# thu-ml/stochastic_gcn

Measured on AMD Instinct MI355X. Metric: training edges/s (SpMM), higher is better.
Workload: dtype f32

## Files before the change

### stochastic_gcn_amd/csrc/sgcn_gemm.hip

```cpp
#include "sgcn_dev.h"
#include "sgcn_bwd.h"

namespace sgcn {

typedef float f16acc __attribute__((ext_vector_type(16)));

constexpr int kTM = 32, kTN = 128, kTK = 32;

struct GemmArgs {
    const float* A; int64_t lda;
    const float* B; int64_t ldb;
    float* C; int64_t ldc;
    int32_t M, N, K;
    int32_t accumulate;
    int32_t kchunk;
    float* ws;
    const float* offset; const float* scale; float eps; int32_t relu;
    float* xhat; float* rstd;
    int32_t epi;
    const float* A2; int64_t lda2; int32_t a_split;
    DropArgs drop_a;
    DropArgs drop_c;
    int32_t vec_a, vec_b;
    const int32_t* a_gidx;
    const int32_t* a_gidx2;
};

__device__ __forceinline__ float wsum(float v) {
#pragma unroll
    for (int o = 32; o > 0; o >>= 1) v += __shfl_xor(v, o, 64);
    return v;
}

constexpr int kAsFloats = kTM * (kTK + 1), kBsFloats = kTK * (kTN + 4);
constexpr int kGroupFloats = kAsFloats + kBsFloats;

template <bool TA, bool TB, int KG>
__device__ __forceinline__ void gemm_body(const GemmArgs& g, const int bx, const int by, const int bz) {
    extern __shared__ float smem[];
    const int kg = threadIdx.x / kBlock;
    const int tid = threadIdx.x % kBlock, lane = tid & 63, wave = tid >> 6;
    float (*As)[kTK + 1] = reinterpret_cast<float (*)[kTK + 1]>(smem + kg * kGroupFloats);
    float (*Bs)[kTN + 4] = reinterpret_cast<float (*)[kTN + 4]>(smem + kg * kGroupFloats + kAsFloats);
    const int m0 = bx * kTM, n0 = by * kTN;
    const int kbeg = bz * g.kchunk;
    const int kend = min(g.K, kbeg + g.kchunk);
    f16acc acc = {};
    float ra[4], rb[16];
    float ep_scale[2] = {1.f, 1.f}, ep_offset[2] = {0.f, 0.f};
    if (g.epi == 2) {
#pragma unroll
        for (int e = 0; e < 2; e++) {
            const int c = (threadIdx.x & 63) + e * kWave;
            if (c < g.N) { ep_scale[e] = g.scale[c]; ep_offset[e] = g.offset[c]; }
        }
    }

    auto ld4 = [&](const float* rowp, bool vec, bool rowok, int first, int limit, float* out) {
        if (vec) {
            const bool ok = rowok && first + 3 < limit;
            const float4 v = *reinterpret_cast<const float4*>(rowp + (ok ? first : 0));
            out[0] = ok ? v.x : 0.f; out[1] = ok ? v.y : 0.f; out[2] = ok ? v.z : 0.f; out[3] = ok ? v.w : 0.f;
        } else {
#pragma unroll
            for (int e = 0; e < 4; e++) {
                const bool ok = rowok && first + e < limit;
                const float v = rowp[ok ? first + e : 0];
                out[e] = ok ? v : 0.f;
            }
        }
    };
    const float* arow = nullptr;
    if (!TA) {
        const int row = min(m0 + (tid >> 3), g.M - 1);
        if (g.A2 && row >= g.a_split) {
            const int r2 = row - g.a_split;
            arow = g.A2 + (int64_t)(g.a_gidx2 ? g.a_gidx2[r2] : r2) * g.lda2;
        } else {
            arow = g.A + (int64_t)(g.a_gidx ? g.a_gidx[row] : row) * g.lda;
        }
    }
    auto fetch = [&](int k0) {
        if (!TA) {
            const int i = tid >> 3, kq = (tid & 7) * 4, row = m0 + i;
            ld4(arow, g.vec_a, row < g.M, k0 + kq, kend, ra);
            if (g.drop_a.on) {
#pragma unroll
                for (int e = 0; e < 4; e++) ra[e] *= drop_factor(g.drop_a, row, k0 + kq + e);
            }
        } else {
            const int kk = tid >> 3, iq = (tid & 7) * 4, k = k0 + kk, kc = min(k, kend - 1);
            const int64_t ak = g.a_gidx ? g.a_gidx[kc] : kc;
            ld4(g.A + ak * g.lda, g.vec_a, k < kend, m0 + iq, g.M, ra);
            if (g.drop_a.on) {
#pragma unroll
                for (int e = 0; e < 4; e++) ra[e] *= drop_factor(g.drop_a, k, m0 + iq + e);
            }
        }
        if (!TB) {
#pragma unroll
            for (int r = 0; r < 4; r++) {
                const int kk = (tid >> 5) + 8 * r, jq = (tid & 31) * 4, k = k0 + kk;
                ld4(g.B + (int64_t)min(k, kend - 1) * g.ldb, g.vec_b, k < kend, n0 + jq, g.N, rb + r * 4);
            }
        } else {
#pragma unroll
            for (int r = 0; r < 4; r++) {
                const int j = (tid >> 3) + 32 * r, kq = (tid & 7) * 4, col = n0 + j;
                ld4(g.B + (int64_t)min(col, g.N - 1) * g.ldb, g.vec_b, col < g.N, k0 + kq, kend, rb + r * 4);
            }
        }
    };
    auto stage = [&]() {
        if (!TA) {
            const int i = tid >> 3, kq = (tid & 7) * 4;
#pragma unroll
            for (int e = 0; e < 4; e++) As[i][kq + e] = ra[e];
        } else {
            const int kk = tid >> 3, iq = (tid & 7) * 4;
#pragma unroll
            for (int e = 0; e < 4; e++) As[iq + e][kk] = ra[e];
        }
        if (!TB) {
#pragma unroll
            for (int r = 0; r < 4; r++) {
                const int kk = (tid >> 5) + 8 * r, jq = (tid & 31) * 4;
                *reinterpret_cast<float4*>(&Bs[kk][jq]) = make_float4(rb[r * 4], rb[r * 4 + 1], rb[r * 4 + 2], rb[r * 4 + 3]);
            }
        } else {
#pragma unroll
            for (int r = 0; r < 4; r++) {
                const int j = (tid >> 3) + 32 * r, kq = (tid & 7) * 4;
#pragma unroll
                for (int e = 0; e < 4; e++) Bs[kq + e][j] = rb[r * 4 + e];
            }
        }
    };

    const int iters = ((kend - kbeg + kTK - 1) / kTK + KG - 1) / KG;
    if (iters > 0) fetch(kbeg + kg * kTK);
    for (int it = 0; it < iters; it++) {
        const int k0 = kbeg + (it * KG + kg) * kTK;
        stage();
        __syncthreads();
        if (it + 1 < iters) fetch(k0 + KG * kTK);
        const int fi = lane & 31, fk = lane >> 5;
#pragma unroll
        for (int kk2 = 0; kk2 < kTK / 2; kk2++) {
            const float a = As[fi][kk2 * 2 + fk];
            const float b = Bs[kk2 * 2 + fk][wave * 32 + fi];
            acc = __builtin_amdgcn_mfma_f32_32x32x2f32(a, b, acc, 0, 0, 0);
        }
        __syncthreads();
    }

    const int cj = wave * 32 + (lane & 31);
    if (KG > 1) {
        if (kg > 0) {
#pragma unroll
            for (int r = 0; r < 16; r++) Bs[(r & 3) + 8 * (r >> 2) + 4 * (lane >> 5)][cj] = acc[r];
        }
        __syncthreads();
        if (kg == 0) {
            for (int o = 1; o < KG; o++) {
                float (*P)[kTN + 4] = reinterpret_cast<float (*)[kTN + 4]>(smem + o * kGroupFloats + kAsFloats);
#pragma unroll
                for (int r = 0; r < 16; r++) acc[r] += P[(r & 3) + 8 * (r >> 2) + 4 * (lane >> 5)][cj];
            }
        }
    }
    if (g.epi == 0) {
        if (kg != 0) return;
        float* base = g.ws ? g.ws + (int64_t)bz * g.M * g.N : g.C;
        const int64_t ld = g.ws ? g.N : g.ldc;
        const bool add = !g.ws && g.accumulate;
#pragma unroll
        for (int r = 0; r < 16; r++) {
            const int row = m0 + (r & 3) + 8 * (r >> 2) + 4 * (lane >> 5), col = n0 + cj;
            if (row < g.M && col < g.N) {
                float* p = base + (int64_t)row * ld + col;
                float v = acc[r];
                if (g.drop_c.on) v *= drop_factor(g.drop_c, row, col);
                *p = add ? *p + v : v;
            }
        }
        return;
    }
    float (*Cs)[kTN + 4] = reinterpret_cast<float (*)[kTN + 4]>(smem + kAsFloats);
    if (KG > 1) __syncthreads();
    if (kg == 0) {
#pragma unroll
        for (int r = 0; r < 16; r++) Cs[(r & 3) + 8 * (r >> 2) + 4 * (lane >> 5)][cj] = acc[r];
    }
    __syncthreads();
    for (int rr = kg * (kBlock / kWave) + wave; rr < kTM; rr += KG * (kBlock / kWave)) {
        const int row = m0 + rr;
        if (row >= g.M) break;
        float* yr = g.C + (int64_t)row * g.ldc;
        if (g.epi == 1) {
            for (int c = lane; c < g.N; c += kWave) { const float v = Cs[rr][c]; yr[c] = g.relu ? fmaxf(v, 0.f) : v; }
            continue;
        }
        float s = 0.f;
        for (int c = lane; c < g.N; c += kWave) s += Cs[rr][c];
        const float mean = wsum(s) / (float)g.N;
        float q = 0.f;
        for (int c = lane; c < g.N; c += kWave) { const float t = Cs[rr][c] - mean; q += t * t; }
        const float rs = rsqrtf(wsum(q) / (float)g.N + g.eps);
        if (lane == 0) g.rstd[row] = rs;
        float* hr = g.xhat + (int64_t)row * g.N;
#pragma unroll
        for (int e = 0; e < 2; e++) {
            const int c = lane + e * kWave;
            if (c < g.N) {
                const float h = (Cs[rr][c] - mean) * rs;
                hr[c] = h;
                const float v = h * ep_scale[e] + ep_offset[e];
                yr[c] = g.relu ? fmaxf(v, 0.f) : v;
            }
        }
    }
}

template <bool TA, bool TB, int KG>
__global__ __launch_bounds__(kBlock * KG) void gemm_kernel(GemmArgs g) {
    gemm_body<TA, TB, KG>(g, (int)blockIdx.x, (int)blockIdx.y, (int)blockIdx.z);
}

struct GemmGroup {
    GemmArgs g[kMaxGroup];
    int32_t first[kMaxGroup + 1];
    int32_t gx[kMaxGroup], gy[kMaxGroup];
    int32_t n;
};

template <bool TA, bool TB, int KG>
__global__ __launch_bounds__(kBlock * KG) void gemm_group_kernel(GemmGroup G) {
    const int b = (int)blockIdx.x;
    int j = 0;
#pragma unroll
    for (int q = 1; q < kMaxGroup; q++) j += (q < G.n && b >= G.first[q]) ? 1 : 0;
    const int l = b - G.first[j];
    const int gx = G.gx[j], gy = G.gy[j];
    gemm_body<TA, TB, KG>(G.g[j], l % gx, (l / gx) % gy, l / (gx * gy));
}

__global__ void splitk_reduce_kernel(const float* __restrict__ ws, int32_t S, int32_t M, int32_t N,
                                     float* __restrict__ C, int64_t ldc, int32_t accumulate) {
    const int64_t i = (int64_t)blockIdx.x * blockDim.x + threadIdx.x;
    const int64_t mn = (int64_t)M * N;
    if (i >= mn) return;
    float s = 0.f;
    for (int z = 0; z < S; z++) s += ws[(int64_t)z * mn + i];
    float* p = C + (i / N) * ldc + (i % N);
    *p = accumulate ? *p + s : s;
}

__global__ void dense_bwd_reduce_kernel(ReduceJob j, int32_t gemm_blocks, const float* __restrict__ ln_partial,
                                        int32_t nblk, int32_t d, float* __restrict__ doffset,
                                        float* __restrict__ dscale, int32_t ln_accumulate) {
    if ((int)blockIdx.x < gemm_blocks) {
        const int64_t i = (int64_t)blockIdx.x * blockDim.x + threadIdx.x;
        const int64_t mn = (int64_t)j.M * j.N;
        if (i >= mn) return;
        float s = 0.f;
        for (int z = 0; z < j.S; z++) s += j.ws[(int64_t)z * mn + i];
        float* p = j.C + (i / j.N) * j.ldc + (i % j.N);
        *p = j.accumulate ? *p + s : s;
    } else {
        ln_param_reduce_cols32(ln_partial, nblk, d, doffset, dscale, (int)blockIdx.x - gemm_blocks, ln_accumulate != 0);
    }
}

__global__ void dense_bwd_reduce_multi_kernel(ReduceMulti R) { reduce_multi_body(R, (int)blockIdx.x, nullptr); }

__global__ __launch_bounds__(kBlock) void splitk_ln_act_kernel(const float* __restrict__ ws, int32_t S,
                                                               GemmArgs g) {
    const int lane = threadIdx.x & 63;
    const int64_t row = (int64_t)blockIdx.x * (kBlock / kWave) + threadIdx.x / kWave;
    if (row >= g.M) return;
    const int64_t mn = (int64_t)g.M * g.N;
    float v[2];
    float sc[2] = {1.f, 1.f}, of[2] = {0.f, 0.f};
    if (g.epi == 2) {
#pragma unroll
        for (int e = 0; e < 2; e++) {
            const int c = lane + e * kWave;
            if (c < g.N) { sc[e] = g.scale[c]; of[e] = g.offset[c]; }
        }
    }
#pragma unroll
    for (int e = 0; e < 2; e++) {
        const int c = lane + e * kWave;
        float s = 0.f;
        if (c < g.N)
            for (int z = 0; z < S; z++) s += ws[(int64_t)z * mn + row * g.N + c];
        v[e] = s;
    }
    float* yr = g.C + row * g.ldc;
    if (g.epi == 2) {
        const float mean = wsum(v[0] + v[1]) / (float)g.N;
        float q = 0.f;
#pragma unroll
        for (int e = 0; e < 2; e++) if (lane + e * kWave < g.N) { const float t = v[e] - mean; q += t * t; }
// ... 93 lines not shown
    }
    if (d.drop.on) { x[0] *= drop_factor(d.drop, (int)row, lane); x[1] *= drop_factor(d.drop, (int)row, lane + kWave); }
    const int c0 = lane < d.N ? lane : 0, c1 = lane + kWave < d.N ? lane + kWave : 0;
    float a0[2] = {0.f, 0.f}, a1[2] = {0.f, 0.f};
    for (int s0 = 0; s0 * 32 < K2; s0++) {
        const int gi = d.kg > 1 ? (s0 & 1) : 0;
        const float xs = s0 < 2 ? x[0] : x[1];
        const int kb = s0 * 32, lb = kb & (kWave - 1);
        const float* wk = wl + kb * d.N;
        float p0 = a0[gi], p1 = a1[gi];
        if (kb + 32 <= K2) {
#pragma unroll
            for (int q = 0; q < 4; q++) {
                float w0[8], w1[8];
#pragma unroll
                for (int u = 0; u < 8; u++) { w0[u] = wk[(q * 8 + u) * d.N + c0]; w1[u] = wk[(q * 8 + u) * d.N + c1]; }
#pragma unroll
                for (int u = 0; u < 8; u++) {
                    const float xv = __int_as_float(__builtin_amdgcn_readlane(__float_as_int(xs), lb + q * 8 + u));
                    p0 = fmaf(xv, w0[u], p0); p1 = fmaf(xv, w1[u], p1);
                }
            }
        } else {
            for (int kk = 0; kb + kk < K2; kk++) {
                const float xv = __int_as_float(__builtin_amdgcn_readlane(__float_as_int(xs), lb + kk));
                p0 = fmaf(xv, wk[kk * d.N + c0], p0); p1 = fmaf(xv, wk[kk * d.N + c1], p1);
            }
        }
        a0[gi] = p0; a1[gi] = p1;
    }
    const float z[2] = {d.kg > 1 ? a0[0] + a0[1] : a0[0], d.kg > 1 ? a1[0] + a1[1] : a1[0]};
    float* y2 = d.Y + row * d.ldy;
    if (d.epi != 2) {
#pragma unroll
        for (int e = 0; e < 2; e++) {
            const int c = lane + e * kWave;
            if (c < d.N) y2[c] = (d.epi == 1 && d.relu) ? fmaxf(z[e], 0.f) : z[e];
        }
        return;
    }
    float s = 0.f;
#pragma unroll
    for (int e = 0; e < 2; e++) if (lane + e * kWave < d.N) s += z[e];
    const float mean = wsum(s) / (float)d.N;
    float q = 0.f;
#pragma unroll
    for (int e = 0; e < 2; e++) if (lane + e * kWave < d.N) { const float t = z[e] - mean; q += t * t; }
    const float rs = rsqrtf(wsum(q) / (float)d.N + d.eps);
    if (lane == 0) d.rstd[row] = rs;
#pragma unroll
    for (int e = 0; e < 2; e++) {
        const int c = lane + e * kWave;
        if (c < d.N) {
            const float h = (z[e] - mean) * rs;
            d.xhat[row * d.N + c] = h;
            const float y = h * sc2[e] + of2[e];
            y2[c] = d.relu ? fmaxf(y, 0.f) : y;
        }
    }
}

}

using namespace sgcn;

static int split_factor(int M, int N, int K) {
    const int tiles = ((M + kTM - 1) / kTM) * ((N + kTN - 1) / kTN);
    int s = 256 / std::max(tiles, 1);
    const int min_steps = tune_get("gemm_min_steps") > 0 ? tune_get("gemm_min_steps") : 3;
    s = std::min(s, K / (min_steps * kTK));
    return std::max(s, 1);
}

template <bool TA, bool TB, int KG>
static void launch_one(const GemmArgs& g, dim3 grid, hipStream_t st) {
    const size_t lds = (size_t)KG * kGroupFloats * sizeof(float);
    static bool raised = false;
    if (lds > 64 * 1024 && !raised) {
        (void)hipFuncSetAttribute(reinterpret_cast<const void*>(&gemm_kernel<TA, TB, KG>),
                                  hipFuncAttributeMaxDynamicSharedMemorySize, (int)lds);
        raised = true;
    }
    hipLaunchKernelGGL((gemm_kernel<TA, TB, KG>), grid, dim3(kBlock * KG), lds, st, g);
}

template <bool TA, bool TB>
static void launch_kg(const GemmArgs& g, dim3 grid, int kgroups, hipStream_t st) {
    if (kgroups >= 4) launch_one<TA, TB, 4>(g, grid, st);
    else if (kgroups == 2) launch_one<TA, TB, 2>(g, grid, st);
    else launch_one<TA, TB, 1>(g, grid, st);
}

struct GemmPlan { dim3 grid; int kgroups, S, epi; };

static GemmPlan prepare_gemm(GemmArgs& g, float* ws, int ta = 0, int tb = 0) {
    auto al = [](const void* p, int64_t ld) { return p && ((uintptr_t)p % 16 == 0) && (ld % 4 == 0); };
    g.vec_a = al(g.A, g.lda) && (!g.A2 || al(g.A2, g.lda2)) && (ta ? g.M : g.K) % 4 == 0;
    g.vec_b = al(g.B, g.ldb) && (tb ? g.K : g.N) % 4 == 0;
    int S = ws ? split_factor(g.M, g.N, g.K) : 1;
    g.kchunk = ((g.K + S - 1) / S + kTK - 1) / kTK * kTK;
    S = g.K > 0 ? (g.K + g.kchunk - 1) / g.kchunk : 1;
    if (g.K == 0) g.kchunk = kTK;
    g.ws = S > 1 ? ws : nullptr;
    GemmPlan p;
    p.epi = g.epi;
    p.S = S;
    if (S > 1) g.epi = 0;
    p.grid = dim3((unsigned)((g.M + kTM - 1) / kTM), (unsigned)((g.N + kTN - 1) / kTN), (unsigned)S);
    const int steps = (std::min(g.kchunk, g.K) + kTK - 1) / kTK;
    const int blocks = (int)(p.grid.x * p.grid.y * p.grid.z);
    p.kgroups = (blocks <= 128 && steps >= 8) ? 4 : ((blocks <= 256 && steps >= 4) ? 2 : 1);
    return p;
}

namespace sgcn {
void gemm_fwd_shape(int M, int N, int K, int* S, int* kgroups, int* kchunk) {
    GemmArgs g{};
    g.M = M; g.N = N; g.K = K;
    float dummy;
    const GemmPlan p = prepare_gemm(g, sgcn_gemm_ws_floats(M, N, K) > 0 ? &dummy : nullptr);
    *S = p.S; *kgroups = p.kgroups;
    if (kchunk) *kchunk = g.kchunk;
}
}

static void launch_prepared(const GemmArgs& g, const GemmPlan& p, int ta, int tb, hipStream_t st) {
    if (!ta && !tb) launch_kg<false, false>(g, p.grid, p.kgroups, st);
    else if (ta && !tb) launch_kg<true, false>(g, p.grid, p.kgroups, st);
    else if (!ta && tb) launch_kg<false, true>(g, p.grid, p.kgroups, st);
    else launch_kg<true, true>(g, p.grid, p.kgroups, st);
}

static int launch_gemm(GemmArgs g, int ta, int tb, float* ws, hipStream_t st, ReduceJob* defer = nullptr) {
    if (defer) defer->pending = 0;
    const GemmPlan p = prepare_gemm(g, ws, ta, tb);
    const int S = p.S, epi = p.epi;
    launch_prepared(g, p, ta, tb, st);
    if (S > 1 && epi != 0) {
        g.epi = epi;
        const unsigned rb = (unsigned)((g.M + (kBlock / kWave) - 1) / (kBlock / kWave));
        hipLaunchKernelGGL(splitk_ln_act_kernel, dim3(rb), dim3(kBlock), 0, st, g.ws, S, g);
    } else if (S > 1 && defer) {
        *defer = ReduceJob{g.ws, S, g.M, g.N, g.C, g.ldc, g.accumulate, 1};
    } else if (S > 1) {
        const int64_t mn = (int64_t)g.M * g.N;
        hipLaunchKernelGGL(splitk_reduce_kernel, dim3((unsigned)((mn + 255) / 256)), dim3(256), 0, st,
                           g.ws, S, g.M, g.N, g.C, g.ldc, g.accumulate);
    }
    SGCN_HIP_TRY(hipGetLastError());
    return SGCN_OK;
}

extern "C" int64_t sgcn_gemm_ws_floats(int32_t M, int32_t N, int32_t K) {
    if (M <= 0 || N <= 0 || K <= 0) return 0;
    const int S = split_factor(M, N, K);
    return S > 1 ? (int64_t)S * M * N : 0;
}

extern "C" int sgcn_gemm_f32(int32_t trans_a, int32_t trans_b, int32_t M, int32_t N, int32_t K,
                             const float* A, int64_t lda, const float* B, int64_t ldb, float* C,
                             int64_t ldc, int32_t accumulate, float* ws,
                             const sgcn_dropout_t* drop_a, const sgcn_dropout_t* drop_c, void* stream) {
    SGCN_REQUIRE(M >= 0 && N >= 0 && K >= 0, "gemm: negative size");
    if (M == 0 || N == 0) return SGCN_OK;
    SGCN_REQUIRE(C && (K == 0 || (A && B)), "gemm: null operand");
    GemmArgs g{};
    g.A = A; g.lda = lda; g.B = B; g.ldb = ldb; g.C = C; g.ldc = ldc;
    g.M = M; g.N = N; g.K = K; g.accumulate = accumulate; g.epi = 0;
    g.drop_a = drop_args(drop_a);
    g.drop_c = drop_args(drop_c);
    SGCN_REQUIRE(!g.drop_a.on || g.drop_a.width == (trans_a ? M : K), "gemm: drop_a width must be the stored A's row length");
    SGCN_REQUIRE(!g.drop_c.on || g.drop_c.width == N, "gemm: drop_c width must be N");
    if (g.drop_c.on) ws = nullptr;
    return launch_gemm(g, trans_a, trans_b, ws, (hipStream_t)stream);
}


namespace sgcn {
int dense_fwd_pair(int32_t M, int32_t N, int32_t K, const float* X, int64_t ldx, const float* X2, int64_t ldx2, int32_t split,
                   const float* W, int64_t ldw, const float* offset, const float* scale, float eps, int32_t relu, float* Y,
                   int64_t ldy, float* xhat, float* rstd, const sgcn_dropout_t* drop, float* ws, const int32_t* gidx,
                   const int32_t* gidx2, int32_t N2, const float* W2, int64_t ldw2, const float* offset2, const float* scale2,
                   float eps2, int32_t relu2, float* Y2, int64_t ldy2, float* xhat2, float* rstd2, const sgcn_dropout_t* drop2,
                   void* stream, int* fused) {
    *fused = 0;
    if (M <= 0 || N <= 0 || N > kTN || N2 <= 0 || N2 > kTN || !ws || !W2 || !Y2 || ldw2 != N2 || ldy != N) return SGCN_OK;
    const int norm = (offset && scale) ? 1 : 0, norm2 = (offset2 && scale2) ? 1 : 0;
    if ((norm && !(xhat && rstd)) || (norm2 && !(xhat2 && rstd2))) return SGCN_OK;
    GemmArgs g{};
    g.A = X; g.lda = ldx; g.B = W; g.ldb = ldw; g.C = Y; g.ldc = ldy;
    g.M = M; g.N = N; g.K = K; g.offset = offset; g.scale = scale; g.eps = eps; g.relu = relu;
    g.xhat = xhat; g.rstd = rstd; g.epi = norm ? 2 : (relu ? 1 : 0);
    g.A2 = X2; g.lda2 = ldx2; g.a_split = split;
    g.a_gidx = gidx; g.a_gidx2 = gidx2;
    g.drop_a = drop_args(drop);
    const GemmPlan p = prepare_gemm(g, ws);
    int S2 = 0, kg2 = 0;
    gemm_fwd_shape(M, N2, N, &S2, &kg2, nullptr);
    if (p.S <= 1 || S2 != 1 || kg2 > 2 || (size_t)N * N2 * sizeof(float) > 64 * 1024 || (N * N2) % 4 || !aligned16(W2)) return SGCN_OK;
    SGCN_REQUIRE(!g.drop_a.on || g.drop_a.width == K, "dense_fwd: dropout width must be K");
    RowDense d{};
    d.W = W2; d.ldw = ldw2; d.N = N2; d.kg = kg2; d.offset = offset2; d.scale = scale2; d.eps = eps2; d.relu = relu2;
    d.epi = norm2 ? 2 : (relu2 ? 1 : 0);
    d.drop = drop_args(drop2);
    SGCN_REQUIRE(!d.drop.on || d.drop.width == N, "dense_fwd: the second layer's dropout width must be its input width");
    d.Y = Y2; d.ldy = ldy2; d.xhat = xhat2; d.rstd = rstd2;
    hipStream_t st = (hipStream_t)stream;
    launch_prepared(g, p, 0, 0, st);
    g.epi = p.epi;
// ... 356 lines not shown
```

### stochastic_gcn_amd/csrc/sgcn_spmm.hip

```cpp
#include "sgcn_dev.h"
#include <cstring>

namespace sgcn {

namespace {
int g_tune_nv = 0;
int g_tune_unroll = 0;
int g_tune_slabmajor = 1;
int g_tune_cs_round = 0;
int g_tune_cs_unroll = 0;
int g_tune_cs_pace = 0;
int g_tune_cs_slack = 0;
int g_tune_cs_noextra = 0;
int g_tune_step_overlap = 1;
int g_tune_step_fuse = 127;
int g_tune_cs_g2_wide = 0;
int g_tune_cs_nowarp = 0;
int g_tune_cs_last_pct = 80;
int g_tune_gemm_min_steps = 0;
int g_tune_gemm_mb16_slice_k = 0;
int g_tune_lds_wave_bias = 100;
int g_tune_lds_mix = 1;
int g_tune_lds_dbg = 0;
thread_local int tl_step_overlap = -1, tl_step_fuse = -1;
}

void step_mode_override(int overlap, int fuse) { tl_step_overlap = overlap; tl_step_fuse = fuse; }

int tune_get(const char* key) {
    if (!strcmp(key, "spmm_nv")) return g_tune_nv;
    if (!strcmp(key, "spmm_unroll")) return g_tune_unroll;
    if (!strcmp(key, "spmm_slabmajor")) return g_tune_slabmajor;
    if (!strcmp(key, "cs_round")) return g_tune_cs_round;
    if (!strcmp(key, "cs_unroll")) return g_tune_cs_unroll;
    if (!strcmp(key, "cs_pace")) return g_tune_cs_pace;
    if (!strcmp(key, "cs_slack")) return g_tune_cs_slack;
    if (!strcmp(key, "cs_noextra")) return g_tune_cs_noextra;
    if (!strcmp(key, "step_overlap")) return tl_step_overlap >= 0 ? tl_step_overlap : g_tune_step_overlap;
    if (!strcmp(key, "step_fuse")) return tl_step_fuse >= 0 ? tl_step_fuse : g_tune_step_fuse;
    if (!strcmp(key, "cs_g2_wide")) return g_tune_cs_g2_wide;
    if (!strcmp(key, "cs_nowarp")) return g_tune_cs_nowarp;
    if (!strcmp(key, "cs_last_pct")) return g_tune_cs_last_pct;
    if (!strcmp(key, "gemm_min_steps")) return g_tune_gemm_min_steps;
    if (!strcmp(key, "gemm_mb16_slice_k")) return g_tune_gemm_mb16_slice_k;
    if (!strcmp(key, "lds_wave_bias")) return g_tune_lds_wave_bias;
    if (!strcmp(key, "lds_mix")) return g_tune_lds_mix;
    if (!strcmp(key, "lds_dbg")) return g_tune_lds_dbg;
    return -1;
}

struct SpmmArgs {
    const int32_t* rowptr;
    const int32_t* col;
    const float* val;
    const sgcn_seg_t* seg;
    int64_t nseg;
    int64_t nsegblk;
    const void* B;
    int64_t ldb;
    const int32_t* gidx;
    const float* rscale;
    const float* cscale;
    float* C;
    int64_t ldc;
    float beta;
    int32_t d;
    int32_t nvec;
    float* ws;
    int64_t ldw;
    int32_t slabmajor;
    const float* add;
    int64_t ldadd;
    int32_t add_rows;
};

template <int VW>
__device__ __forceinline__ void epilogue_store(const SpmmArgs& a, int row, int vi,
                                               typename Vec<VW>::type acc, float rs) {
    float* out = a.C + (int64_t)row * a.ldc + (int64_t)vi * VW;
    typename Vec<VW>::type r = acc * rs;
    const int left = a.d - vi * VW;
    if (a.beta != 0.f) {
        if (left >= VW) r += a.beta * vload<VW>(out);
        else {
#pragma unroll
            for (int e = 0; e < VW; e++)
                if (e < left) {
                    if constexpr (VW == 1) r += a.beta * out[0]; else r[e] += a.beta * out[e];
                }
        }
    }
    if (a.add && row < a.add_rows) {
        const float* ad = a.add + (int64_t)row * a.ldadd + (int64_t)vi * VW;
        if (left >= VW) r += vload<VW>(ad);
        else {
#pragma unroll
            for (int e = 0; e < VW; e++)
                if (e < left) {
                    if constexpr (VW == 1) r += ad[0]; else r[e] += ad[e];
                }
        }
    }
    if (left >= VW) vstore<VW>(out, r);
    else vstore_head<VW>(out, r, left);
}

template <int G, int NV, int VW, int U, class BT>
__global__ __launch_bounds__(kBlock) void spmm_seg_kernel(SpmmArgs a) {
    typedef typename Vec<VW>::type VT;
    typedef typename HRaw<BT, VW>::type RT;
    constexpr bool kB16 = !std::is_same<BT, float>::value;
    constexpr int GPB = kBlock / G;
    const int lig = threadIdx.x & (G - 1);
    const int gib = threadIdx.x / G;

    int slab;
    int64_t sblk;
    if (a.slabmajor) { slab = (int)(blockIdx.x / a.nsegblk); sblk = blockIdx.x % a.nsegblk; }
    else { const int nslab = (int)(gridDim.x / a.nsegblk); slab = blockIdx.x % nslab; sblk = blockIdx.x / nslab; }
    const int64_t s = sblk * GPB + gib;
    if (s >= a.nseg) return;

    int row, start, end, slot;
    if (a.seg) {
        const sgcn_seg_t sg = a.seg[s];
        row = sg.row; start = sg.start; end = sg.end; slot = sg.slot;
// ... 71 lines not shown
        for (int k = 0; k < NV; k++)
            if (act[k]) vstore<VW>(w + (int64_t)k * G * VW, acc[k]);
    }
}

template <int VW>
__global__ __launch_bounds__(kBlock) void spmm_fix_kernel(SpmmArgs a, const sgcn_fix_t* fix,
                                                          int64_t nfix) {
    typedef typename Vec<VW>::type VT;
    const int nvblk = (a.nvec + kBlock - 1) / kBlock;
    const int64_t f = blockIdx.x / nvblk;
    if (f >= nfix) return;
    const sgcn_fix_t fx = fix[f];
    const int vi = (int)(blockIdx.x % nvblk) * kBlock + threadIdx.x;
    if (vi >= a.nvec) return;
    const float* w = a.ws + (int64_t)fx.first_slot * a.ldw + (int64_t)vi * VW;
    VT acc = vzero<VW>();
    for (int q = 0; q < fx.nslots; q++) acc += vload<VW>(w + (int64_t)q * a.ldw);
    const float rs = a.rscale ? a.rscale[fx.row] : 1.0f;
    epilogue_store<VW>(a, fx.row, vi, acc, rs);
}

template <int G, int NV, int VW, int U, class BT>
static void launch_seg(const SpmmArgs& a, int64_t nblocks, hipStream_t st) {
    hipLaunchKernelGGL((spmm_seg_kernel<G, NV, VW, U, BT>), dim3((unsigned)nblocks), dim3(kBlock), 0, st, a);
}

template <int VW, int U, class BT>
static bool dispatch_gnv(int G, int NV, const SpmmArgs& a, int64_t nblocks, hipStream_t st) {
    switch (G) {
        case 8: launch_seg<8, 1, VW, U, BT>(a, nblocks, st); return true;
        case 16: launch_seg<16, 1, VW, U, BT>(a, nblocks, st); return true;
        case 32: launch_seg<32, 1, VW, U, BT>(a, nblocks, st); return true;
        case 64:
            switch (NV) {
                case 1: launch_seg<64, 1, VW, U, BT>(a, nblocks, st); return true;
                case 2: launch_seg<64, 2, VW, U, BT>(a, nblocks, st); return true;
                case 3: launch_seg<64, 3, VW, U, BT>(a, nblocks, st); return true;
                case 4: launch_seg<64, 4, VW, U, BT>(a, nblocks, st); return true;
            }
    }
    return false;
}

template <int VW, class BT>
static bool dispatch_u(int U, int G, int NV, const SpmmArgs& a, int64_t nblocks, hipStream_t st) {
    switch (U) {
        case 2: return dispatch_gnv<VW, 2, BT>(G, NV, a, nblocks, st);
        case 4: return dispatch_gnv<VW, 4, BT>(G, NV, a, nblocks, st);
        case 8: return dispatch_gnv<VW, 8, BT>(G, NV, a, nblocks, st);
    }
    return false;
}

int group_lanes(int nvec) {
    if (nvec <= 8) return 8;
    if (nvec <= 16) return 16;
    if (nvec <= 32) return 32;
    return 64;
}

}

using namespace sgcn;

extern "C" int64_t sgcn_tune_get(const char* key) { return key ? tune_get(key) : -1; }

extern "C" int sgcn_tune(const char* key, int64_t value) {
    if (!key) return fail(SGCN_ERR_INVALID, "sgcn_tune: null key");
    if (!strcmp(key, "spmm_nv")) { SGCN_REQUIRE(value >= 0 && value <= 4, "spmm_nv in 0..4"); g_tune_nv = (int)value; return SGCN_OK; }
    if (!strcmp(key, "spmm_unroll")) {
        SGCN_REQUIRE(value == 0 || value == 2 || value == 4 || value == 8, "spmm_unroll in {0,2,4,8}");
        g_tune_unroll = (int)value; return SGCN_OK;
    }
    if (!strcmp(key, "spmm_slabmajor")) { g_tune_slabmajor = value != 0; return SGCN_OK; }
    if (!strcmp(key, "cs_pace")) { SGCN_REQUIRE(value >= 0, "cs_pace >= 0"); g_tune_cs_pace = (int)value; return SGCN_OK; }
    if (!strcmp(key, "cs_slack")) { SGCN_REQUIRE(value >= 0, "cs_slack >= 0"); g_tune_cs_slack = (int)value; return SGCN_OK; }
    if (!strcmp(key, "cs_noextra")) { g_tune_cs_noextra = value != 0; return SGCN_OK; }
    if (!strcmp(key, "step_overlap")) { g_tune_step_overlap = value != 0; return SGCN_OK; }
    if (!strcmp(key, "step_fuse")) { SGCN_REQUIRE(value >= 0 && value <= 127, "step_fuse in 0..127"); g_tune_step_fuse = (int)value; return SGCN_OK; }
    if (!strcmp(key, "cs_g2_wide")) { g_tune_cs_g2_wide = value != 0; return SGCN_OK; }
    if (!strcmp(key, "cs_nowarp")) { g_tune_cs_nowarp = value != 0; return SGCN_OK; }
    if (!strcmp(key, "gemm_min_steps")) { g_tune_gemm_min_steps = (int)value; return SGCN_OK; }
    if (!strcmp(key, "gemm_mb16_slice_k")) {
        SGCN_REQUIRE(value >= 0 && value <= 0x7fffffff, "gemm_mb16_slice_k >= 0");
        g_tune_gemm_mb16_slice_k = (int)value; return SGCN_OK;
    }
    if (!strcmp(key, "lds_wave_bias")) { SGCN_REQUIRE(value >= 50 && value <= 300, "lds_wave_bias in 50..300 (per cent)"); g_tune_lds_wave_bias = (int)value; return SGCN_OK; }
    if (!strcmp(key, "lds_mix")) { g_tune_lds_mix = value != 0; return SGCN_OK; }
    if (!strcmp(key, "lds_dbg")) { g_tune_lds_dbg = (int)value; return SGCN_OK; }
    if (!strcmp(key, "cs_last_pct")) { SGCN_REQUIRE(value >= 0 && value <= 100, "cs_last_pct in [0, 100]"); g_tune_cs_last_pct = (int)value; return SGCN_OK; }
    if (!strcmp(key, "cs_round")) { SGCN_REQUIRE(value >= 0, "cs_round >= 0"); g_tune_cs_round = (int)value; return SGCN_OK; }
    if (!strcmp(key, "cs_unroll")) {
        SGCN_REQUIRE(value == 0 || value == 4 || value == 8, "cs_unroll in {0,4,8}");
        g_tune_cs_unroll = (int)value; return SGCN_OK;
    }
    return fail(SGCN_ERR_INVALID, "sgcn_tune: unknown key '%s'", key);
}

template <class BT>
static int spmm_csr_add(const int32_t* rowptr, const int32_t* col, const float* val,
                        int32_t M, int32_t K, int32_t d, const BT* B, int64_t ldb,
                        const int32_t* gidx, const float* rscale, const float* cscale,
                        float* C, int64_t ldc, float beta, const sgcn_plan_t* plan,
                        const float* add, int64_t ldadd, int32_t add_rows, void* stream) {
    constexpr bool kB16 = !std::is_same<BT, float>::value;
    SGCN_REQUIRE(M >= 0 && K >= 0 && d >= 0, "spmm: negative size");
    if (M == 0 || d == 0) return SGCN_OK;
    SGCN_REQUIRE(rowptr && C && (B || K == 0), "spmm: null operand");
    SGCN_REQUIRE(ldb >= d && ldc >= d, "spmm: leading dimension smaller than d");
    if (kB16) {
        SGCN_REQUIRE(ldb % 8 == 0, "spmm: a bfloat16 operand needs ldb %% 8 == 0 (ldb %lld, d %d)", (long long)ldb, d);
        SGCN_REQUIRE(aligned16(B), "spmm: a bfloat16 operand needs a 16-byte aligned base");
    }
    hipStream_t st = (hipStream_t)stream;

    SpmmArgs a{};
    a.rowptr = rowptr; a.col = col; a.val = val;
    a.B = B; a.ldb = ldb; a.gidx = gidx; a.rscale = rscale; a.cscale = cscale;
    a.C = C; a.ldc = ldc; a.beta = beta; a.d = d;
    a.nseg = M;
    a.slabmajor = g_tune_slabmajor;
    if (add && add_rows > 0) {
        SGCN_REQUIRE(ldadd >= d && add_rows <= M, "spmm: bad addend");
        a.add = add; a.ldadd = ldadd; a.add_rows = add_rows;
    }
    if (plan) {
        SGCN_REQUIRE(plan->dev_seg && plan->nseg >= M, "spmm: malformed plan");
        a.seg = plan->dev_seg; a.nseg = plan->nseg;
        a.ws = plan->dev_ws; a.ldw = ((int64_t)d + 3) / 4 * 4;
        if (plan->nfix > 0) {
            SGCN_REQUIRE(plan->dev_fix && plan->dev_ws, "spmm: plan with split rows needs dev_fix/dev_ws");
            SGCN_REQUIRE(plan->ws_elems >= plan->nslots * a.ldw,
                         "spmm: workspace too small (%lld < %lld floats)", (long long)plan->ws_elems,
                         (long long)(plan->nslots * a.ldw));
        }
    }
    const int vw = pick_vw(d, {kB16 ? nullptr : (const void*)B, C, plan ? plan->dev_ws : nullptr, a.add},
                           {ldb, ldc, a.add ? a.ldadd : ldc});
    a.nvec = (d + vw - 1) / vw;
    const int G = group_lanes(a.nvec);
    int NV = 1;
    if (G == 64) {
        const int per_wave = (a.nvec + 63) / 64;
        const int nslab0 = (per_wave + 3) / 4;
        NV = (per_wave + nslab0 - 1) / nslab0;
        if (g_tune_nv > 0) NV = g_tune_nv;
    }
    const int nslab = (a.nvec + G * NV - 1) / (G * NV);
    const int U = g_tune_unroll > 0 ? g_tune_unroll : (NV >= 3 ? 4 : 8);
    a.nsegblk = (a.nseg + (kBlock / G) - 1) / (kBlock / G);
    const int64_t nblocks = a.nsegblk * nslab;
    SGCN_REQUIRE(nblocks < (1ll << 31), "spmm: grid too large");

    bool ok = false;
    if (vw == 4) ok = dispatch_u<4, BT>(U, G, NV, a, nblocks, st);
    else if (vw == 2) ok = dispatch_u<2, BT>(U, G, NV, a, nblocks, st);
    else ok = dispatch_u<1, BT>(U, G, NV, a, nblocks, st);
    SGCN_REQUIRE(ok, "spmm: no kernel for G=%d NV=%d U=%d", G, NV, U);
    SGCN_HIP_TRY(hipGetLastError());

    if (plan && plan->nfix > 0) {
        const int64_t nfblk = (int64_t)((a.nvec + kBlock - 1) / kBlock) * plan->nfix;
        SGCN_REQUIRE(nfblk < (1ll << 31), "spmm: too many split rows");
        dim3 grid((unsigned)nfblk);
        if (vw == 4) hipLaunchKernelGGL((spmm_fix_kernel<4>), grid, dim3(kBlock), 0, st, a, plan->dev_fix, plan->nfix);
// ... 43 lines not shown
```

Before: 7.432 billion.

## Add multi-stage LDS ring pipeline for dense GEMM using direct global-to-LDS loads

```diff
diff --git a/profiles/gemm_pipe_probe.py b/profiles/gemm_pipe_probe.py
--- /dev/null
+++ b/profiles/gemm_pipe_probe.py
@@ -0,0 +1,105 @@
+import json
+import os
+import statistics
+import sys
+
+import torch
+
+sys.path.insert(0, os.path.dirname(os.path.dirname(os.path.abspath(__file__))))
+from stochastic_gcn_amd import _ffi, ops
+
+dev = torch.device("cuda:0")
+gen = torch.Generator(device=dev)
+gen.manual_seed(0)
+label = sys.argv[sys.argv.index("--label") + 1] if "--label" in sys.argv else "tree"
+OUT = sys.argv[sys.argv.index("--out") + 1] if "--out" in sys.argv else None
+WINDOWS, REPS = 5, 200
+
+
+def rnd(*s):
+    return torch.randn(*s, device=dev, generator=gen)
+
+
+try:
+    _ffi.tune("gemm_pipe", 1)
+    ARMS = (0, 1)
+except Exception:
+    ARMS = (None,)
+PLUG = torch.randn(6144, 6144, device=dev)
+
+
+def window(fn, reps):
+    e0, e1 = torch.cuda.Event(enable_timing=True), torch.cuda.Event(enable_timing=True)
+    for _ in range(2):
+        torch.mm(PLUG, PLUG)
+    e0.record()
+    for _ in range(reps):
+        fn()
+    e1.record()
+    torch.cuda.synchronize()
+    return e0.elapsed_time(e1) * 1e3 / reps
+
+
+def measure(name, table, fn, reps=REPS):
+    got = {a: [] for a in ARMS}
+    for a in ARMS:
+        if a is not None:
+            _ffi.tune("gemm_pipe", a)
+        for _ in range(10):
+            fn()
+    torch.cuda.synchronize()
+    for _ in range(WINDOWS):
+        for a in ARMS:
+            if a is not None:
+                _ffi.tune("gemm_pipe", a)
+            got[a].append(window(fn, reps))
+    for a in ARMS:
+        v = got[a]
+        rec = {"label": label, "call": name, "table_rows": table, "gemm_pipe": "none" if a is None else a, "windows": WINDOWS,
+               "calls_per_window": reps, "us_min": round(min(v), 2), "us_median": round(statistics.median(v), 2),
+               "us_max": round(max(v), 2)}
+        line = json.dumps(rec)
+        print(line, flush=True)
+        if OUT:
+            with open(OUT, "a") as f:
+                f.write(line + "\n")
+
+
+n, K, N = 1021, 1204, 128
+W = rnd(K, N) * 0.05
+off, sc = rnd(1, N) * 0.1, 1 + rnd(1, N) * 0.1
+dy = rnd(2 * n, N)
+dW = torch.zeros(K, N, device=dev)
+drop = ops.Drop(0.8, ops.dropout_key(1, 0, 0))
+feat = rnd(232965, K)
+SETS = 40
+
+
+def cycle(calls):
+    state = [0]
+
+    def fn():
+        calls[state[0] % len(calls)]()
+        state[0] += 1
+    return fn
+
+
+for rows in (232965, 2 * n):
+    table = feat if rows == 232965 else feat[:rows].clone()
+    nn, tn = [], []
+    for _ in range(SETS):
+        idx = torch.randperm(rows, device=dev, generator=gen)[:2 * n].to(torch.int32)
+        x = ops.GatheredRows(table, idx[:n].contiguous())
+        x2 = ops.GatheredRows(table, idx[n:].contiguous())
+        xa = ops.GatheredRows(table, idx)
+        nn.append(lambda x=x, x2=x2: ops.dense_fwd(x, W, off, sc, True, x2=x2, drop=drop))
+        tn.append(lambda xa=xa: ops.dense_bwd(dy, None, None, None, False, xa, W, dW, need_dx=False, drop=drop))
+    measure("NN first layer 2042 x 1204 -> 128 (+ row-pass reduce)", rows, cycle(nn))
+    measure("TN weight gradient 1204 x 128 over 2042 rows (+ reduce)", rows, cycle(tn))
+if "--big" in sys.argv:
+    M = 232965
+    g = rnd(M, N)
+    measure("NN full graph 232965 x 1204 -> 128", M, lambda: ops.dense_fwd(feat, W, off, sc, True), reps=10)
+    measure("TN full graph 1204 x 128 over 232965 rows", M, lambda: ops.gemm(feat, g, out=dW, trans_a=True), reps=10)
+if ARMS != (None,):
+    _ffi.tune("gemm_pipe", 1)
diff --git a/stochastic_gcn_amd/csrc/sgcn_gemm.hip b/stochastic_gcn_amd/csrc/sgcn_gemm.hip
--- a/stochastic_gcn_amd/csrc/sgcn_gemm.hip
+++ b/stochastic_gcn_amd/csrc/sgcn_gemm.hip
@@ -24,6 +24,7 @@
     int32_t vec_a, vec_b;
     const int32_t* a_gidx;
     const int32_t* a_gidx2;
+    int32_t ring;
 };
 
 __device__ __forceinline__ float wsum(float v) {
@@ -34,6 +35,82 @@
 
 constexpr int kAsFloats = kTM * (kTK + 1), kBsFloats = kTK * (kTN + 4);
 constexpr int kGroupFloats = kAsFloats + kBsFloats;
+
+template <int KG>
+__device__ __forceinline__ void gemm_finish(const GemmArgs& g, f16acc acc, float* smem, const int gstride, const int toff,
+                                            const int bx, const int by, const int bz, const float (&ep_scale)[2],
+                                            const float (&ep_offset)[2]) {
+    const int kg = threadIdx.x / kBlock;
+    const int tid = threadIdx.x % kBlock, lane = tid & 63, wave = tid >> 6;
+    const int m0 = bx * kTM, n0 = by * kTN;
+    float (*Ps)[kTN + 4] = reinterpret_cast<float (*)[kTN + 4]>(smem + kg * gstride + toff);
+    const int cj = wave * 32 + (lane & 31);
+    if (KG > 1) {
+        if (kg > 0) {
+#pragma unroll
+            for (int r = 0; r < 16; r++) Ps[(r & 3) + 8 * (r >> 2) + 4 * (lane >> 5)][cj] = acc[r];
+        }
+        __syncthreads();
+        if (kg == 0) {
+            for (int o = 1; o < KG; o++) {
+                float (*P)[kTN + 4] = reinterpret_cast<float (*)[kTN + 4]>(smem + o * gstride + toff);
+#pragma unroll
+                for (int r = 0; r < 16; r++) acc[r] += P[(r & 3) + 8 * (r >> 2) + 4 * (lane >> 5)][cj];
+            }
+        }
+    }
+    if (g.epi == 0) {
+        if (kg != 0) return;
+        float* base = g.ws ? g.ws + (int64_t)bz * g.M * g.N : g.C;
+        const int64_t ld = g.ws ? g.N : g.ldc;
+        const bool add = !g.ws && g.accumulate;
+#pragma unroll
+        for (int r = 0; r < 16; r++) {
+            const int row = m0 + (r & 3) + 8 * (r >> 2) + 4 * (lane >> 5), col = n0 + cj;
+            if (row < g.M && col < g.N) {
+                float* p = base + (int64_t)row * ld + col;
+                float v = acc[r];
+                if (g.drop_c.on) v *= drop_factor(g.drop_c, row, col);
+                *p = add ? *p + v : v;
+            }
+        }
+        return;
+    }
+    float (*Cs)[kTN + 4] = reinterpret_cast<float (*)[kTN + 4]>(smem + toff);
+    if (KG > 1) __syncthreads();
+    if (kg == 0) {
+#pragma unroll
+        for (int r = 0; r < 16; r++) Cs[(r & 3) + 8 * (r >> 2) + 4 * (lane >> 5)][cj] = acc[r];
+    }
+    __syncthreads();
+    for (int rr = kg * (kBlock / kWave) + wave; rr < kTM; rr += KG * (kBlock / kWave)) {
+        const int row = m0 + rr;
+        if (row >= g.M) break;
+        float* yr = g.C + (int64_t)row * g.ldc;
+        if (g.epi == 1) {
+            for (int c = lane; c < g.N; c += kWave) { const float v = Cs[rr][c]; yr[c] = g.relu ? fmaxf(v, 0.f) : v; }
+            continue;
+        }
+        float s = 0.f;
+        for (int c = lane; c < g.N; c += kWave) s += Cs[rr][c];
+        const float mean = wsum(s) / (float)g.N;
+        float q = 0.f;
+        for (int c = lane; c < g.N; c += kWave) { const float t = Cs[rr][c] - mean; q += t * t; }
+        const float rs = rsqrtf(wsum(q) / (float)g.N + g.eps);
+        if (lane == 0) g.rstd[row] = rs;
+        float* hr = g.xhat + (int64_t)row * g.N;
+#pragma unroll
+        for (int e = 0; e < 2; e++) {
+            const int c = lane + e * kWave;
+            if (c < g.N) {
+                const float h = (Cs[rr][c] - mean) * rs;
+                hr[c] = h;
+                const float v = h * ep_scale[e] + ep_offset[e];
+                yr[c] = g.relu ? fmaxf(v, 0.f) : v;
+            }
+        }
+    }
+}
 
 template <bool TA, bool TB, int KG>
 __device__ __forceinline__ void gemm_body(const GemmArgs& g, const int bx, const int by, const int bz) {
@@ -154,72 +231,204 @@
         __syncthreads();
     }
 
-    const int cj = wave * 32 + (lane & 31);
-    if (KG > 1) {
-        if (kg > 0) {
-#pragma unroll
-            for (int r = 0; r < 16; r++) Bs[(r & 3) + 8 * (r >> 2) + 4 * (lane >> 5)][cj] = acc[r];
-        }
-        __syncthreads();
-        if (kg == 0) {
-            for (int o = 1; o < KG; o++) {
-                float (*P)[kTN + 4] = reinterpret_cast<float (*)[kTN + 4]>(smem + o * kGroupFloats + kAsFloats);
-#pragma unroll
-                for (int r = 0; r < 16; r++) acc[r] += P[(r & 3) + 8 * (r >> 2) + 4 * (lane >> 5)][cj];
-            }
-        }
-    }
-    if (g.epi == 0) {
-        if (kg != 0) return;
-        float* base = g.ws ? g.ws + (int64_t)bz * g.M * g.N : g.C;
-        const int64_t ld = g.ws ? g.N : g.ldc;
-        const bool add = !g.ws && g.accumulate;
-#pragma unroll
-        for (int r = 0; r < 16; r++) {
-            const int row = m0 + (r & 3) + 8 * (r >> 2) + 4 * (lane >> 5), col = n0 + cj;
-            if (row < g.M && col < g.N) {
-                float* p = base + (int64_t)row * ld + col;
-                float v = acc[r];
-                if (g.drop_c.on) v *= drop_factor(g.drop_c, row, col);
-                *p = add ? *p + v : v;
-            }
-        }
-        return;
-    }
-    float (*Cs)[kTN + 4] = reinterpret_cast<float (*)[kTN + 4]>(smem + kAsFloats);
-    if (KG > 1) __syncthreads();
-    if (kg == 0) {
-#pragma unroll
-        for (int r = 0; r < 16; r++) Cs[(r & 3) + 8 * (r >> 2) + 4 * (lane >> 5)][cj] = acc[r];
-    }
+    gemm_finish<KG>(g, acc, smem, kGroupFloats, kAsFloats, bx, by, bz, ep_scale, ep_offset);
+}
+
+constexpr int kPipeA = kTM * kTK, kPipeB = kTK * kTN, kPipeStage = kPipeA + kPipeB;
+constexpr int kPipeDma = 5;
+constexpr int kPipeMaxRing = 8;
+constexpr int kPipeIdx = 2048;
+
+template <int N> __device__ __forceinline__ void pipe_wait() { asm volatile("s_waitcnt vmcnt(%0)" :: "n"(N) : "memory"); }
+__device__ __forceinline__ void pipe_wait_behind(int behind) {
+    switch (behind) {
+        case 0: pipe_wait<0>(); break;
+        case 1: pipe_wait<kPipeDma>(); break;
+        case 2: pipe_wait<2 * kPipeDma>(); break;
+        case 3: pipe_wait<3 * kPipeDma>(); break;
+        case 4: pipe_wait<4 * kPipeDma>(); break;
+        case 5: pipe_wait<5 * kPipeDma>(); break;
+        case 6: pipe_wait<6 * kPipeDma>(); break;
+        default: pipe_wait<7 * kPipeDma>(); break;
+    }
+}
+__device__ __forceinline__ void pipe_barrier() {
+    asm volatile("s_waitcnt lgkmcnt(0)" ::: "memory");
+    __builtin_amdgcn_s_barrier();
+    asm volatile("" ::: "memory");
+}
+typedef float pf4 __attribute__((ext_vector_type(4)));
+__device__ __forceinline__ uint32_t pipe_lds_addr(const void* p) {
+    return (uint32_t)(uintptr_t)(const __attribute__((address_space(3))) void*)p;
+}
+template <int OFF> __device__ __forceinline__ float pipe_rd32(uint32_t addr) {
+    float v;
+    asm volatile("ds_read_b32 %0, %1 offset:%2" : "=v"(v) : "v"(addr), "n"(OFF));
+    return v;
+}
+__device__ __forceinline__ int pipe_rd32i(uint32_t addr) {
+    int v;
+    asm volatile("ds_read_b32 %0, %1\n\ts_waitcnt lgkmcnt(0)" : "=v"(v) : "v"(addr));
+    return v;
+}
+__device__ __forceinline__ pf4 pipe_rd128(uint32_t addr) {
+    pf4 v;
+    asm volatile("ds_read_b128 %0, %1" : "=v"(v) : "v"(addr));
+    return v;
+}
+__device__ __forceinline__ void pipe_wr128(uint32_t addr, pf4 v) {
+    asm volatile("ds_write_b128 %0, %1" :: "v"(addr), "v"(v) : "memory");
+}
+__device__ __forceinline__ void pipe_dma16(const float* src, float* lds_wave_base) {
+    __builtin_amdgcn_global_load_lds((const __attribute__((address_space(1))) void*)src,
+                                     (__attribute__((address_space(3))) void*)lds_wave_base, 16, 0, 0);
+}
+
+template <bool TA, int KG>
+__device__ __forceinline__ void gemm_pipe_body(const GemmArgs& g, const int bx, const int by, const int bz) {
+    extern __shared__ __attribute__((aligned(1024))) float smem[];
+    const int kg = threadIdx.x / kBlock;
+    const int tid = threadIdx.x % kBlock, lane = tid & 63, wave = tid >> 6;
+    const int D = g.ring, gstride = D * kPipeStage;
+    float* ring = smem + kg * gstride;
+    int* kidx = reinterpret_cast<int*>(smem + KG * gstride);
+    const int m0 = bx * kTM, n0 = by * kTN;
+    const int kbeg = bz * g.kchunk;
+    const int kend = min(g.K, kbeg + g.kchunk);
+    f16acc acc = {};
+    float ep_scale[2] = {1.f, 1.f}, ep_offset[2] = {0.f, 0.f};
+    if (g.epi == 2) {
+#pragma unroll
+        for (int e = 0; e < 2; e++) {
+            const int c = (threadIdx.x & 63) + e * kWave;
+            if (c < g.N) { ep_scale[e] = g.scale[c]; ep_offset[e] = g.offset[c]; }
+        }
+    }
+    const int iters = ((kend - kbeg + kTK - 1) / kTK + KG - 1) / KG;
+    const int ai = tid >> 3, aslot = tid & 7;
+    const float* arow = nullptr;
+    int achunk = 0;
+    bool a_in = true;
+    if (!TA) {
+        const int row = min(m0 + ai, g.M - 1);
+        if (g.A2 && row >= g.a_split) {
+            const int r2 = row - g.a_split;
+            arow = g.A2 + (int64_t)(g.a_gidx2 ? g.a_gidx2[r2] : r2) * g.lda2;
+        } else {
+            arow = g.A + (int64_t)(g.a_gidx ? g.a_gidx[row] : row) * g.lda;
+        }
+        achunk = aslot ^ ((ai >> 1) & 7);
+    } else {
+        achunk = aslot;
+        a_in = m0 + aslot * 4 + 3 < g.M;
+        if (g.a_gidx) {
+            for (int q = threadIdx.x; q < kend - kbeg; q += kBlock * KG) kidx[q] = g.a_gidx[kbeg + q];
+            __syncthreads();
+        }
+    }
+    const int bcol = n0 + (tid & 31) * 4;
+    const float* bsrc = g.B + (bcol + 3 < g.N ? bcol : 0);
+    const int bk = tid >> 5;
+    const bool dropt = g.drop_a.on && (TA || m0 < g.drop_a.rows);
+
+    auto request = [&](int st) {
+        float* sa = ring + (st % D) * kPipeStage;
+        float* sb = sa + kPipeA;
+        const int k0 = kbeg + (st * KG + kg) * kTK;
+        if (!TA) {
+            const int k = k0 + achunk * 4;
+            pipe_dma16(arow + (k + 3 < kend ? k : 0), sa + wave * 256);
+        } else {
+            const int kc = max(min(k0 + ai, kend - 1), kbeg);
+            const int64_t ak = g.a_gidx ? pipe_rd32i(pipe_lds_addr(kidx + (kc - kbeg))) : kc;
+            pipe_dma16(g.A + ak * g.lda + (a_in ? m0 + achunk * 4 : 0), sa + wave * 256);
+        }
+#pragma unroll
+        for (int r = 0; r < 4; r++) {
+            const int kc = max(min(k0 + bk + 8 * r, kend - 1), kbeg);
+            pipe_dma16(bsrc + (int64_t)kc * g.ldb, sb + r * 1024 + wave * 256);
+        }
+    };
+
+    int issued = 0;
+    for (; issued < D && issued < iters; issued++) request(issued);
+    const int fi = lane & 31, fk = lane >> 5;
+    const int aswz = (fi >> 1) & 7;
+    const uint32_t ring_addr = pipe_lds_addr(ring);
+    for (int it = 0; it < iters; it++) {
+        pipe_wait_behind(issued - 1 - it);
+        pipe_barrier();
+        if (it > 0 && issued < iters) { request(issued); issued++; }
+        const uint32_t sa = ring_addr + (uint32_t)((it % D) * kPipeStage * (int)sizeof(float)), sb = sa + kPipeA * (uint32_t)sizeof(float);
+        const int k0 = kbeg + (it * KG + kg) * kTK;
+        if (dropt) {
+            pf4 v = pipe_rd128(sa + tid * 16);
+            asm volatile("s_waitcnt lgkmcnt(0)" : "+v"(v));
+            if (!TA) {
+                const int row = m0 + ai, k = k0 + achunk * 4;
+                v.x *= drop_factor(g.drop_a, row, k); v.y *= drop_factor(g.drop_a, row, k + 1);
+                v.z *= drop_factor(g.drop_a, row, k + 2); v.w *= drop_factor(g.drop_a, row, k + 3);
+            } else {
+                const int k = k0 + ai, m = m0 + achunk * 4;
+                v.x *= drop_factor(g.drop_a, k, m); v.y *= drop_factor(g.drop_a, k, m + 1);
+                v.z *= drop_factor(g.drop_a, k, m + 2); v.w *= drop_factor(g.drop_a, k, m + 3);
+            }
+            pipe_wr128(sa + tid * 16, v);
+            pipe_barrier();
+        }
+        float fa[16], fb[16];
+        const uint32_t bfrag = sb + (uint32_t)((fk * kTN + wave * 32 + fi) * 4);
+#define SGCN_PIPE_RD16(dst, base, stride) \
+        dst[0] = pipe_rd32<0 * stride>(base); dst[1] = pipe_rd32<1 * stride>(base); dst[2] = pipe_rd32<2 * stride>(base); \
+        dst[3] = pipe_rd32<3 * stride>(base); dst[4] = pipe_rd32<4 * stride>(base); dst[5] = pipe_rd32<5 * stride>(base); \
+        dst[6] = pipe_rd32<6 * stride>(base); dst[7] = pipe_rd32<7 * stride>(base); dst[8] = pipe_rd32<8 * stride>(base); \
+        dst[9] = pipe_rd32<9 * stride>(base); dst[10] = pipe_rd32<10 * stride>(base); dst[11] = pipe_rd32<11 * stride>(base); \
+        dst[12] = pipe_rd32<12 * stride>(base); dst[13] = pipe_rd32<13 * stride>(base); dst[14] = pipe_rd32<14 * stride>(base); \
+        dst[15] = pipe_rd32<15 * stride>(base);
+#define SGCN_PIPE_TIE16(x) "+v"(x[0]), "+v"(x[1]), "+v"(x[2]), "+v"(x[3]), "+v"(x[4]), "+v"(x[5]), "+v"(x[6]), "+v"(x[7]), "+v"(x[8]), \
+        "+v"(x[9]), "+v"(x[10]), "+v"(x[11]), "+v"(x[12]), "+v"(x[13]), "+v"(x[14]), "+v"(x[15])
+        if (!TA) {
+            pf4 va[8];
+            const uint32_t arowaddr = sa + (uint32_t)(fi * kTK * 4);
+#pragma unroll
+            for (int c = 0; c < 8; c++) va[c] = pipe_rd128(arowaddr + (uint32_t)((c ^ aswz) << 4));
+            SGCN_PIPE_RD16(fb, bfrag, 2 * kTN * 4)
+            asm volatile("s_waitcnt lgkmcnt(0)" : "+v"(va[0]), "+v"(va[1]), "+v"(va[2]), "+v"(va[3]), "+v"(va[4]), "+v"(va[5]),
+                         "+v"(va[6]), "+v"(va[7]));
+#pragma unroll
+            for (int c = 0; c < 8; c++) {
+                fa[2 * c] = fk ? va[c].y : va[c].x;
+                fa[2 * c + 1] = fk ? va[c].w : va[c].z;
+            }
+        } else {
+            const uint32_t afrag = sa + (uint32_t)((fk * kTM + fi) * 4);
+            SGCN_PIPE_RD16(fa, afrag, 2 * kTM * 4)
+            SGCN_PIPE_RD16(fb, bfrag, 2 * kTN * 4)
+            asm volatile("s_waitcnt lgkmcnt(0)" : SGCN_PIPE_TIE16(fa));
+        }
+        asm volatile("" : SGCN_PIPE_TIE16(fb));
+#undef SGCN_PIPE_RD16
+#undef SGCN_PIPE_TIE16
+        if (k0 + kTK > kend) {
+            const int klim = kend - k0 - fk;
+#pragma unroll
+            for (int kk2 = 0; kk2 < 16; kk2++) {
+                const bool ok = kk2 * 2 < klim;
+                fa[kk2] = ok ? fa[kk2] : 0.f;
+                fb[kk2] = ok ? fb[kk2] : 0.f;
+            }
+        }
+#pragma unroll
+        for (int kk2 = 0; kk2 < 16; kk2++) acc = __builtin_amdgcn_mfma_f32_32x32x2f32(fa[kk2], fb[kk2], acc, 0, 0, 0);
+    }
+    pipe_wait<0>();
     __syncthreads();
-    for (int rr = kg * (kBlock / kWave) + wave; rr < kTM; rr += KG * (kBlock / kWave)) {
-        const int row = m0 + rr;
-        if (row >= g.M) break;
-        float* yr = g.C + (int64_t)row * g.ldc;
-        if (g.epi == 1) {
-            for (int c = lane; c < g.N; c += kWave) { const float v = Cs[rr][c]; yr[c] = g.relu ? fmaxf(v, 0.f) : v; }
-            continue;
-        }
-        float s = 0.f;
-        for (int c = lane; c < g.N; c += kWave) s += Cs[rr][c];
-        const float mean = wsum(s) / (float)g.N;
-        float q = 0.f;
-        for (int c = lane; c < g.N; c += kWave) { const float t = Cs[rr][c] - mean; q += t * t; }
-        const float rs = rsqrtf(wsum(q) / (float)g.N + g.eps);
-        if (lane == 0) g.rstd[row] = rs;
-        float* hr = g.xhat + (int64_t)row * g.N;
-#pragma unroll
-        for (int e = 0; e < 2; e++) {
-            const int c = lane + e * kWave;
-            if (c < g.N) {
-                const float h = (Cs[rr][c] - mean) * rs;
-                hr[c] = h;
-                const float v = h * ep_scale[e] + ep_offset[e];
-                yr[c] = g.relu ? fmaxf(v, 0.f) : v;
-            }
-        }
-    }
+    gemm_finish<KG>(g, acc, smem, gstride, 0, bx, by, bz, ep_scale, ep_offset);
+}
+
+template <bool TA, int KG>
+__global__ __launch_bounds__(kBlock * KG) void gemm_pipe_kernel(GemmArgs g) {
+    gemm_pipe_body<TA, KG>(g, (int)blockIdx.x, (int)blockIdx.y, (int)blockIdx.z);
 }
 
 template <bool TA, bool TB, int KG>
@@ -479,6 +688,53 @@
         raised = true;
     }
     hipLaunchKernelGGL((gemm_kernel<TA, TB, KG>), grid, dim3(kBlock * KG), lds, st, g);
+}
+
+constexpr size_t kPipeLdsCap = 160 * 1024;
+static int pipe_ring_depth(int64_t blocks, int kgroups, int steps_per_group, size_t idx_bytes) {
+    const int64_t per_cu = std::max<int64_t>(1, (blocks + 255) / 256);
+    const int64_t budget = (int64_t)(kPipeLdsCap / (size_t)per_cu) - (int64_t)idx_bytes;
+    int64_t d = budget / ((int64_t)kgroups * kPipeStage * (int64_t)sizeof(float));
+    d = std::min<int64_t>(d, std::min(kPipeMaxRing, std::max(steps_per_group, 2)));
+    return (int)std::max<int64_t>(d, 2);
+}
+static size_t pipe_lds_bytes(int kgroups, int ring, size_t idx_bytes) {
+    return (size_t)kgroups * ring * kPipeStage * sizeof(float) + idx_bytes;
+}
+static int plan_kg(int kgroups) { return kgroups >= 4 ? 4 : (kgroups == 2 ? 2 : 1); }
+
+static bool pipe_plan(GemmArgs& g, dim3 grid, int kgroups, int ta, int tb) {
+    g.ring = 0;
+    if (tune_get("gemm_pipe") == 0 || tb || !g.vec_a || !g.vec_b || g.K <= 0) return false;
+    const bool idx = ta && g.a_gidx;
+    if (idx && g.kchunk > kPipeIdx) return false;
+    const int KG = plan_kg(kgroups);
+    const int steps = (std::min(g.kchunk, g.K) + kTK - 1) / kTK;
+    const size_t idx_bytes = ta ? kPipeIdx * sizeof(int32_t) : 0;
+    const int64_t blocks = (int64_t)grid.x * grid.y * grid.z;
+    const int ring = pipe_ring_depth(blocks, KG, (steps + KG - 1) / KG, idx_bytes);
+    if (pipe_lds_bytes(KG, ring, idx_bytes) > kPipeLdsCap) return false;
+    g.ring = ring;
+    return true;
+}
+
+template <bool TA, int KG>
+static void launch_pipe_one(const GemmArgs& g, dim3 grid, hipStream_t st) {
+    const size_t lds = pipe_lds_bytes(KG, g.ring, TA ? kPipeIdx * sizeof(int32_t) : 0);
+    static bool raised = false;
+    if (lds > 64 * 1024 && !raised) {
+        (void)hipFuncSetAttribute(reinterpret_cast<const void*>(&gemm_pipe_kernel<TA, KG>),
+                                  hipFuncAttributeMaxDynamicSharedMemorySize, (int)kPipeLdsCap);
+        raised = true;
+    }
+    hipLaunchKernelGGL((gemm_pipe_kernel<TA, KG>), grid, dim3(kBlock * KG), lds, st, g);
+}
+
+template <bool TA>
+static void launch_pipe_kg(const GemmArgs& g, dim3 grid, int kgroups, hipStream_t st) {
+    if (kgroups >= 4) launch_pipe_one<TA, 4>(g, grid, st);
+    else if (kgroups == 2) launch_pipe_one<TA, 2>(g, grid, st);
+    else launch_pipe_one<TA, 1>(g, grid, st);
 }
 
 template <bool TA, bool TB>
@@ -521,7 +777,13 @@
 }
 }
 
-static void launch_prepared(const GemmArgs& g, const GemmPlan& p, int ta, int tb, hipStream_t st) {
+static void launch_prepared(const GemmArgs& g0, const GemmPlan& p, int ta, int tb, hipStream_t st) {
+    GemmArgs g = g0;
+    if (pipe_plan(g, p.grid, p.kgroups, ta, tb)) {
+        if (ta) launch_pipe_kg<true>(g, p.grid, p.kgroups, st);
+        else launch_pipe_kg<false>(g, p.grid, p.kgroups, st);
+        return;
+    }
     if (!ta && !tb) launch_kg<false, false>(g, p.grid, p.kgroups, st);
     else if (ta && !tb) launch_kg<true, false>(g, p.grid, p.kgroups, st);
     else if (!ta && tb) launch_kg<false, true>(g, p.grid, p.kgroups, st);
diff --git a/stochastic_gcn_amd/csrc/sgcn_spmm.hip b/stochastic_gcn_amd/csrc/sgcn_spmm.hip
--- a/stochastic_gcn_amd/csrc/sgcn_spmm.hip
+++ b/stochastic_gcn_amd/csrc/sgcn_spmm.hip
@@ -18,6 +18,7 @@
 int g_tune_cs_nowarp = 0;
 int g_tune_cs_last_pct = 80;
 int g_tune_gemm_min_steps = 0;
+int g_tune_gemm_pipe = 1;
 int g_tune_gemm_mb16_slice_k = 0;
 int g_tune_lds_wave_bias = 100;
 int g_tune_lds_mix = 1;
@@ -42,6 +43,7 @@
     if (!strcmp(key, "cs_nowarp")) return g_tune_cs_nowarp;
     if (!strcmp(key, "cs_last_pct")) return g_tune_cs_last_pct;
     if (!strcmp(key, "gemm_min_steps")) return g_tune_gemm_min_steps;
+    if (!strcmp(key, "gemm_pipe")) return g_tune_gemm_pipe;
     if (!strcmp(key, "gemm_mb16_slice_k")) return g_tune_gemm_mb16_slice_k;
     if (!strcmp(key, "lds_wave_bias")) return g_tune_lds_wave_bias;
     if (!strcmp(key, "lds_mix")) return g_tune_lds_mix;
@@ -279,6 +281,11 @@
     if (!strcmp(key, "cs_g2_wide")) { g_tune_cs_g2_wide = value != 0; return SGCN_OK; }
     if (!strcmp(key, "cs_nowarp")) { g_tune_cs_nowarp = value != 0; return SGCN_OK; }
     if (!strcmp(key, "gemm_min_steps")) { g_tune_gemm_min_steps = (int)value; return SGCN_OK; }
+    if (!strcmp(key, "gemm_pipe")) {
+        SGCN_REQUIRE(value == 0 || value == 1, "tune: gemm_pipe is 0 (register-staged) or 1 (automatic)");
+        g_tune_gemm_pipe = (int)value;
+        return SGCN_OK;
+    }
     if (!strcmp(key, "gemm_mb16_slice_k")) {
         SGCN_REQUIRE(value >= 0 && value <= 0x7fffffff, "gemm_mb16_slice_k >= 0");
         g_tune_gemm_mb16_slice_k = (int)value; return SGCN_OK;
```

New measurement: 7.419 billion. Within noise of the previous version (-0.2%).
